# grero/HMMSpikeSorter.jl

Hardware: AMD Instinct MI355X
Metric: Msamples/sec (Viterbi + forward-backward), K=4 L=60 HMM (higher is better)
Workload: dtype f64; 1 GPU; K=4 L=60 HMM (reference N=4, K=60: 237 states), 10000000-sample single channel per GPU: one Viterbi decode + one Baum-Welch E-step (forward-backward + sufficient statistics + M-step finish); channels=1, samples_per_channel=10000000, states=237, engine=wave, block=4928, halo=295, chains=2030, seed=1234, pooled_allreduce=False

## Files before the change

### hmmspikesorter.jl_amd/csrc/wave_common.h

```cpp
#pragma once
#include <hip/hip_runtime.h>
#include <stdint.h>
#include <cmath>
#include <cstdlib>
#include <cstring>
#include <string>
#include <vector>

#include "hmmsort_internal.h"
#include "ring_common.h"

namespace hmmsort {

constexpr double kScFloor = -700.0;

struct WaveGeom {
    int64_t T;
    int C;
    int N, L;
    int W;
    int RB;
    int B;
    int Hw;
    int He;
// ... 132 lines not shown
    bool uc = true;
    int pre_rows = 0;
    bool sweeps = false;
    bool logdl = false;
    int ft = 0;
    bool gs = false;
    int gsum = kGsumNone;
    int nt = 0, ngrp = 0;
    bool decode = false;
    bool redo = false;
    bool tight = false;
    bool light = false;
    int spw = 0;
};

inline WavePick wave_pick(const WaveDev *r, int call)
{
    const WaveGeom &g = r->g;
    const int N = g.N, L = g.L;
    WavePick p;
    p.N = N; p.call = call;
    p.uc = r->uniform_cx || N > kWaveMaxPerSource;
    p.pre_rows = wave_pre_rows(N);
    p.sweeps = call != kWaveCallDecode;
    p.decode = call == kWaveCallDecode || call == kWaveCallDecodeEstep;
    if (p.sweeps) {
        p.logdl = N > 8;
        p.gs = call == kWaveCallPosteriors;
        const bool generic = getenv("HMMSORT_GSUM_GENERIC") != nullptr;
        const bool fuse4 = N == 3 || N == 4, fuse8 = N >= 5 && N <= 8;
        const bool sep = generic || p.gs || getenv("HMMSORT_GSUM_SEPARATE") != nullptr;
        p.ft = sep ? 0 : (fuse4 && L <= 64) ? 1 : (fuse8 && r->uniform_cx && L <= 64) ? 2
               : (fuse8 && r->uniform_cx && L <= 128) ? 4 : 0;
        if (p.gs) p.gsum = kGsumNone;
        else if (p.ft > 0) p.gsum = kGsumFused;
        else if (generic) p.gsum = kGsumGeneric;
        else {
            static const int nt_big = getenv("HMMSORT_GSUM_TILES") ? atoi(getenv("HMMSORT_GSUM_TILES")) : 16;
            const int want = nt_big >= 16 ? 16 : (nt_big >= 8 ? 8 : 4);
            const int np = N <= 1 ? 1 : (N <= 2 ? 2 : (N <= 4 ? 4 : (N <= 8 ? 8 : 16)));
            const int lpt = 16 * (16 / np);
            const int ntx = (L + lpt - 1) / lpt;
            p.gsum = kGsumMx;
            p.nt = N > 8 ? (ntx <= 4 ? 4 : (ntx <= 8 ? (want < 8 ? want : 8) : want)) : (ntx < 4 ? ntx : 4);
            p.ngrp = (ntx + p.nt - 1) / p.nt;
        }
    }
    if (p.decode) {
        const bool beside = call == kWaveCallDecodeEstep;
        p.redo = g.nch > 1;
        p.tight = N <= 4 && beside;
        p.light = g.backtrace == 2 || (g.backtrace == 0 && beside);
        p.spw = wave_bt_spw(N);
    }
    return p;
}

__device__ __forceinline__ double wave_bcast(double v, int lane)
{
    const int lo = __builtin_amdgcn_readlane(__double2loint(v), lane);
    const int hi = __builtin_amdgcn_readlane(__double2hiint(v), lane);
    return __hiloint2double(hi, lo);
}

template <int CTRL, int ROWMASK>
__device__ __forceinline__ double dpp_mov(double old, double v)
{
    const int lo = __builtin_amdgcn_update_dpp(__double2loint(old), __double2loint(v), CTRL, ROWMASK, 0xF, false);
    const int hi = __builtin_amdgcn_update_dpp(__double2hiint(old), __double2hiint(v), CTRL, ROWMASK, 0xF, false);
    return __hiloint2double(hi, lo);
}

__device__ __forceinline__ double lane_prev(double v, double carry)
{
    return dpp_mov<0x138, 0xF>(carry, v);
}

__device__ __forceinline__ void scan_maxplus(double &a, double &b)
{
#define HS_MP_STEP(CTRL, RM)                                                      \
    {                                                                             \
        const double al = dpp_mov<CTRL, RM>(0.0, a), bl = dpp_mov<CTRL, RM>(-INFINITY, b); \
        b = fmax(bl + a, b);                                                      \
        a = al + a;                                                               \
    }
    HS_MP_STEP(0x111, 0xF) HS_MP_STEP(0x112, 0xF) HS_MP_STEP(0x114, 0xF) HS_MP_STEP(0x118, 0xF)
    HS_MP_STEP(0x142, 0xA) HS_MP_STEP(0x143, 0xC)
#undef HS_MP_STEP
}

template <int CTRL, int ROWMASK>
__device__ __forceinline__ float dpp_movf(float old, float v)
{
    return __int_as_float(__builtin_amdgcn_update_dpp(__float_as_int(old), __float_as_int(v), CTRL, ROWMASK, 0xF, false));
}
__device__ __forceinline__ void scan_maxplus_f32(float &a, float &b)
{
#define HS_MPF_STEP(CTRL, RM)                                                     \
    {                                                                             \
        const float al = dpp_movf<CTRL, RM>(0.0f, a), bl = dpp_movf<CTRL, RM>(-INFINITY, b); \
        b = fmaxf(bl + a, b);                                                     \
        a = al + a;                                                               \
    }
    HS_MPF_STEP(0x111, 0xF) HS_MPF_STEP(0x112, 0xF) HS_MPF_STEP(0x114, 0xF) HS_MPF_STEP(0x118, 0xF)
    HS_MPF_STEP(0x142, 0xA) HS_MPF_STEP(0x143, 0xC)
#undef HS_MPF_STEP
}
__device__ __forceinline__ float lane_prevf(float v, float carry)
{
    return dpp_movf<0x138, 0xF>(carry, v);
}

__device__ __forceinline__ void scan_linear(double &a, double &b)
{
#define HS_LN_STEP(CTRL, RM)                                                      \
    {                                                                             \
        const double al = dpp_mov<CTRL, RM>(1.0, a), bl = dpp_mov<CTRL, RM>(0.0, b); \
        b = __builtin_fma(a, bl, b);                                              \
        a = al * a;                                                               \
    }
    HS_LN_STEP(0x111, 0xF) HS_LN_STEP(0x112, 0xF) HS_LN_STEP(0x114, 0xF) HS_LN_STEP(0x118, 0xF)
    HS_LN_STEP(0x142, 0xA) HS_LN_STEP(0x143, 0xC)
#undef HS_LN_STEP
}

__device__ __forceinline__ double lane_prev_ref(double v, double carry, int lane)
{
    const double s = __shfl_up(v, 1);
    return lane == 0 ? carry : s;
}
__device__ __forceinline__ void scan_maxplus_ref(double &a, double &b, int lane)
{
#pragma unroll
    for (int d = 1; d < 64; d <<= 1) {
        const double al = __shfl_up(a, d), bl = __shfl_up(b, d);
        if (lane >= d) { b = fmax(bl + a, b); a = al + a; }
    }
}
__device__ __forceinline__ void scan_linear_ref(double &a, double &b, int lane)
{
#pragma unroll
    for (int d = 1; d < 64; d <<= 1) {
        const double al = __shfl_up(a, d), bl = __shfl_up(b, d);
        if (lane >= d) { b = __builtin_fma(a, bl, b); a = al * a; }
    }
}

__device__ __forceinline__ const WaveConst *reload_consts(const WaveConst *p)
{
    asm volatile("" : "+s"(p));
    return p;
}

template <int N> constexpr int wave_depth() { return N <= 4 ? 4 : (N <= 8 ? 3 : 2); }
template <int N> constexpr int wave_occ() { return N <= 4 ? 4 : (N <= 8 ? 2 : 1); }

__device__ __forceinline__ double wave_max(double v)
{
#pragma unroll
    for (int o = 32; o > 0; o >>= 1) v = fmax(v, __shfl_xor(v, o));
    return v;
}
__device__ __forceinline__ double wave_sum(double v)
{
#pragma unroll
    for (int o = 32; o > 0; o >>= 1) v += __shfl_xor(v, o);
    return v;
}

__device__ __forceinline__ void wave_lds_order()
{
    __builtin_amdgcn_fence(__ATOMIC_RELEASE, "wavefront");
    __builtin_amdgcn_wave_barrier();
    __builtin_amdgcn_fence(__ATOMIC_ACQUIRE, "wavefront");
}

constexpr int kTieBlk = 512;
constexpr int kTieCap = 65536;
constexpr int kTieWalk = 8192;
constexpr int kTieLanes = 64;
constexpr int kTieTrig = 0;
constexpr int kTieListed = 1;
constexpr int kTieDone = 2;
constexpr int kTieFlips = 3;
constexpr int kTieOpen = 4;
constexpr int kTieTail = 5;
constexpr int kTieLongest = 6;
constexpr int kTieSerial = 7;

__device__ __forceinline__ double wpath_lp(int N, int L, const double *__restrict__ ctab, int xp, int xc)
{
    if (xp == 1) return xc == 1 ? ctab[0] : ctab[1 + (xc - 2) / L];
    const int a = (xp - 2) / L, k = (xp - 2) % L + 1;
    if (k < L) return ctab[1 + 2 * N + N * N + a * L + k];
    if (xc == 1) return ctab[1 + N + a];
    return ctab[1 + 2 * N + a * N + (xc - 2) / L];
}

__device__ __forceinline__ double wave_thr(const WaveGeom &g, const WaveConst &K, const double *__restrict__ ysum, int ch)
{
    const double T = (double)g.T;
    const double s1 = ysum[2 * ch], s2 = ysum[2 * ch + 1];
    const double sq = fmax((s2 - 2.0 * K.mean0 * s1) + T * K.mean0 * K.mean0, 0.0);
    const double mmax = fabs(K.A) * T + sq / K.den + fabs(K.c00) * T + 1.0;
    return (ldexp(16.0 * (double)(g.L + 2), ilogb(mmax) - 52) + 4.0e-9) * g.thr_scale;
}

template <typename F>
int wave_graphed(WaveDev *r, int kind, const void *p0, const void *p1, const void *p2, const void *p3,
                 hipStream_t st, F enqueue)
{
    if (!r->graphs_on || r->prof_on || st == nullptr) return enqueue(st);
    uint64_t key[12] = {(uint64_t)kind, (uint64_t)(uintptr_t)p0, (uint64_t)(uintptr_t)p1, (uint64_t)(uintptr_t)p2,
                        (uint64_t)(uintptr_t)p3, (uint64_t)(uintptr_t)st, (uint64_t)(r->bound_y == p0),
                        (uint64_t)r->uniform_cx, (uint64_t)r->g.own_lo, (uint64_t)r->g.own_hi,
                        (uint64_t)(r->g.first * 2 + r->g.last), (uint64_t)(uint32_t)r->g.tie_debug};
    {
        uint64_t tb;
        static_assert(sizeof(tb) == sizeof(r->g.thr_scale), "");
        memcpy(&tb, &r->g.thr_scale, sizeof(tb));
        key[11] ^= tb << 8;
    }
    for (auto &e : r->graphs)
        if (!memcmp(e.key, key, sizeof(key))) {
            HS_HIP(hipGraphLaunch(e.exec, st));
            return HMMSORT_OK;
        }
    if (hipStreamBeginCapture(st, hipStreamCaptureModeRelaxed) != hipSuccess) {
        (void)hipGetLastError();
        r->graphs_on = false;
        return enqueue(st);
    }
    const int rc = enqueue(st);
    hipGraph_t graph = nullptr;
    const hipError_t e1 = hipStreamEndCapture(st, &graph);
    hipGraphExec_t exec = nullptr;
    if (rc || e1 != hipSuccess || !graph || hipGraphInstantiate(&exec, graph, nullptr, nullptr, 0) != hipSuccess) {
        (void)hipGetLastError();
        if (graph) (void)hipGraphDestroy(graph);
        r->graphs_on = false;
        return rc ? rc : enqueue(st);
    }
    (void)hipGraphDestroy(graph);
    if (r->graphs.size() >= 16) {
        (void)hipGraphExecDestroy(r->graphs.front().exec);
        r->graphs.erase(r->graphs.begin());
    }
    WaveDev::GraphEntry ge;
    memcpy(ge.key, key, sizeof(key));
    ge.exec = exec;
    r->graphs.push_back(ge);
    HS_HIP(hipGraphLaunch(exec, st));
    return HMMSORT_OK;
}

inline size_t wave_zero_bytes(const WaveDev *r, bool decode)
{
    return (size_t)(decode ? 8 + 8 * (int64_t)r->g.C + 2 : 8) * sizeof(int64_t);
}

int wave_create(WaveDev **out, const std::vector<HostModel> &models, int64_t T, int64_t block_req,
                int64_t halo_req);
int wave_set_model(WaveDev *r, int ch, const HostModel &m);
void wave_destroy(WaveDev *r);
int wave_prepare(WaveDev *r, const double *d_y, hipStream_t st);
int wave_bind(WaveDev *r, const double *d_y, hipStream_t st);
int64_t wave_stats_len(const WaveDev *r);
int wave_diagnostics(WaveDev *r, hipStream_t st, int64_t diag[8]);
int wave_profile_read(WaveDev *r, hipStream_t st, std::vector<std::string> &names,
                      std::vector<double> &ms, std::vector<int64_t> &calls);
int wave_viterbi_sweep(WaveDev *r, const double *d_y, hipStream_t st);
int wave_viterbi_post(WaveDev *r, const double *d_y, int16_t *d_x, double *d_ll, hipStream_t st, bool beside);
int wave_viterbi(WaveDev *r, const double *d_y, int16_t *d_x, double *d_ll, hipStream_t st);
int wave_tie_resolve(WaveDev *r, const double *d_y, int16_t *d_x, hipStream_t st);
int wave_tie_stats(WaveDev *r, hipStream_t st, int64_t out[8]);
int wave_estep(WaveDev *r, const double *d_y, double *d_stats, hipStream_t st);
int wave_mstep(WaveDev *r, const double *d_stats, double *d_out, hipStream_t st);
int wave_decode_estep(WaveDev *r, const double *d_y, int16_t *d_x, double *d_ll, double *d_stats,
                      hipStream_t st);
int wave_post_sweeps(WaveDev *r, const double *d_y, hipStream_t st);
int wave_posteriors(WaveDev *r, const double *d_y, double *d_onset, double *d_occ, double *d_silent, double *d_logz,
                    hipStream_t st);
int wave_post_decode(WaveDev *r, int16_t *d_xm, hipStream_t st);
int wave_spike_conf(WaveDev *r, int ch, int a, int qv, int64_t jitter, const int64_t *d_times, int64_t n,
                    double *d_conf, hipStream_t st);
int wave_expected_counts(WaveDev *r, double *counts_out, hipStream_t st);

}
```

### hmmspikesorter.jl_amd/csrc/wave_estep.hip

```cpp
#include <cmath>
#include <type_traits>

#include "fastmath.h"
#include "wave_common.h"

namespace hmmsort {

constexpr double kLn2 = 6.93147180559945286227e-01;
typedef double wg_d4 __attribute__((ext_vector_type(4)));

__device__ __forceinline__ double scale_of(double v, double s)
{
    return v > 0.0 ? s + (double)ilogb(v) * kLn2 : -INFINITY;
}

template <int N>
struct FIn {
    double y;
    double R[N];
};

template <int N>
__device__ __forceinline__ void excl_sums(const double (&t)[N], double (&out)[N])
{
    double pre = 0.0;
#pragma unroll
    for (int a = 0; a < N; a++) { out[a] = pre; pre += t[a]; }
    double suf = 0.0;
#pragma unroll
    for (int a = N - 1; a >= 0; a--) { out[a] += suf; suf += t[a]; }
}

template <int N, bool UC>
__global__ __launch_bounds__(64, N <= 4 ? 3 : (N <= 8 ? 2 : 1)) void kw_fwd(WaveGeom g, const WaveConst *__restrict__ cst,
                                                            const double *__restrict__ y,
                                                            const double *__restrict__ Rf,
                                                            const double *__restrict__ virt,
                                                            double *__restrict__ FA0, double *__restrict__ FV,
                                                            double *__restrict__ FREF, double *__restrict__ fpre,
                                                            double *__restrict__ trash)
{
    constexpr int D = wave_depth<N>();
    constexpr int KSC = 5, KCP0 = 5 + N, KPEND = 5 + 2 * N, KCPX = 5 + 3 * N, KSIZE = 5 + 3 * N + N * N;
    extern __shared__ double lds[];
    const int L = g.L, W = g.W, RB = g.RB, B = g.B;
    constexpr bool LOGDL = N > 8;
    double *KC = lds, *DLv = lds + KSIZE, *DLs = LOGDL ? DLv : lds + KSIZE + N * (RB + 1);
    const int lane = threadIdx.x;
    const int cg = blockIdx.x, ch = cg / g.nch, c = cg % g.nch;
    const int64_t T = g.T;
    const int64_t tc = (int64_t)c * B;
    const int nc = (int)((T - tc) < B ? (T - tc) : B);
    const int64_t tend = tc + nc;
    const double *yc = y + (int64_t)ch * T;
    const double *Rc = Rf + (int64_t)ch * N * T;
    double *FAc = FA0 + (int64_t)ch * T, *FRc = FREF + (int64_t)ch * T, *FVc = FV + (int64_t)ch * N * T;
    const int64_t FR = 1 + (int64_t)L * (N + 1);
    double *rec = fpre + cg * FR;

    if (LOGDL) for (int i = lane; i < N * (RB + 1); i += 64) DLv[i] = -INFINITY;
    else for (int i = lane; i < 2 * N * (RB + 1); i += 64) DLv[i] = 0.0;
    {
        const WaveConst &Kg = cst[ch];
        if (lane == 0) { KC[0] = Kg.sc0; KC[1] = Kg.mean0; KC[2] = 1.0 / Kg.den; KC[3] = Kg.P00; KC[4] = fexp(-Kg.sc0); }
        if (lane < N) { KC[KSC + lane] = Kg.sc[lane]; KC[KCP0 + lane] = Kg.CP0[lane]; KC[KPEND + lane] = Kg.PEND[lane]; }
        if (UC) { if (lane < N) KC[KCPX + lane] = Kg.CPXin[lane]; }
        else for (int i = lane; i < N * N; i += 64) KC[KCPX + i] = Kg.CPXT[i];
    }
    __syncthreads();
    int64_t tinit;
    double M, x = 1.0;
    if (c == 0) {
        tinit = 0;
        for (int i = lane; i < N * L; i += 64) {
            const int a = i / L, j = i % L + 1;
            if (j < L) {
                if (!LOGDL) DLv[a * (RB + 1) + (L - j)] = 1.0;
                DLs[a * (RB + 1) + (L - j)] = virt[((int64_t)ch * N + a) * (L + 1) + j];
            }
        }
        const double d0 = yc[0] - KC[1];
        const double q00 = -((d0 * d0) * KC[2]);
        M = (double)(float)q00;
        x = fexp(q00 - M);
        if (lane < N) {
            const double f0 = fexp(-KC[KSC + lane]);
            if (LOGDL) DLs[lane * (RB + 1) + L] = Rc[(int64_t)lane * T];
            else {
                DLv[lane * (RB + 1) + L] = f0;
                DLs[lane * (RB + 1) + L] = KC[KSC + lane] + Rc[(int64_t)lane * T];
            }
            FVc[(int64_t)lane * T] = f0;
        }
        if (lane == 0) { FAc[0] = q00; FRc[0] = 0.0; }
    } else {
        tinit = tc - g.Hw;
        M = 0.0;
    }
    __syncthreads();

    const int n_total = (int)(tend - 1 - tinit);
    auto load = [&](FIn<N> &d, int off) {
        const int nact = n_total - off < W ? n_total - off : W;
        const int li = lane < nact ? lane : 0;
        int64_t tb = tinit + 1 + off;
        tb = tb < T ? tb : T - 1;
        d.y = (yc + tb)[li];
#pragma unroll
        for (int a = 0; a < N; a++) d.R[a] = (Rc + (int64_t)a * T + tb)[li];
    };
    int rs = (1 + lane) % RB, ws = (L + 1 + lane) % RB;
    auto run = [&](const FIn<N> &d, int off, auto mode_tag) {
        constexpr int MODE = decltype(mode_tag)::value;
        const int nact = n_total - off < W ? n_total - off : W;
        const bool live = lane < nact;
        const int64_t tb = tinit + 1 + off;
        const int64_t t = tb + lane;
        const double sc0 = KC[0];
        double v[N], E[N + 1];
        double e = -INFINITY;
#pragma unroll
        for (int a = 0; a < N; a++) {
            if (LOGDL) {
                v[a] = 1.0;
                E[a] = live ? DLs[a * (RB + 1) + rs] + sc0 : -INFINITY;
                e = fmax(e, E[a]);
            } else {
                v[a] = live ? DLv[a * (RB + 1) + rs] : 0.0;
                E[a] = DLs[a * (RB + 1) + rs] + sc0;
                e = fmax(e, scale_of(v[a], E[a]));
            }
        }
        const double dd = d.y - KC[1];
        const double q0 = -((dd * dd) * KC[2]);
        float fa = live ? (float)(sc0 + q0) : 0.0f;
        float fb = live ? (float)(e + q0) : -INFINITY;
        scan_maxplus_f32(fa, fb);
        const float Mf = (float)M;
        const float Mtf = fmaxf(Mf + fa, fb);
        const double Mt = (double)Mtf;
        const double Mprev = (double)lane_prevf(Mtf, Mf);
        const double ref = Mt - q0;
        E[N] = (Mprev + sc0) - ref;
#pragma unroll
        for (int a = 0; a < N; a++) E[a] = v[a] > 0.0 ? fmin(E[a] - ref, 700.0) : -INFINITY;
        fexp_n<N + 1>(E);
        const double E0 = E[N];
        double Ea[N];
        double al = E0 * KC[3], be = 0.0;
#pragma unroll
        for (int a = 0; a < N; a++) {
            Ea[a] = LOGDL ? E[a] : v[a] * E[a];
            be = __builtin_fma(Ea[a], KC[KPEND + a], be);
        }
        al = live ? al : 1.0;
        be = live ? be : 0.0;
        scan_linear(al, be);
        const double xt = __builtin_fma(al, x, be);
        const double xprev = lane_prev(xt, x);
        const double einv = KC[4];
        const double base = (xprev * E0) * einv;
        double u[N];
        if (UC) {
            double tb_[N], ex[N];
#pragma unroll
            for (int a = 0; a < N; a++) tb_[a] = Ea[a] * einv;
            excl_sums<N>(tb_, ex);
#pragma unroll
            for (int a = 0; a < N; a++) u[a] = __builtin_fma(ex[a], KC[KCPX + a], base * KC[KCP0 + a]);
        } else {
#pragma unroll
            for (int a = 0; a < N; a++) {
                double su = base * KC[KCP0 + a];
#pragma unroll
                for (int b = 0; b < N; b++)
                    if (b != a) su = __builtin_fma(Ea[b] * einv, KC[KCPX + a * N + b], su);
                u[a] = su;
                __builtin_amdgcn_sched_barrier(0);
            }
        }
        const int wsl = live ? ws : RB;
        if (LOGDL) {
            double lu[N];
#pragma unroll
            for (int a = 0; a < N; a++) lu[a] = u[a];
            flog_n<N>(lu);
#pragma unroll
            for (int a = 0; a < N; a++) DLs[a * (RB + 1) + wsl] = ((ref + KC[KSC + a]) + d.R[a]) + (u[a] > 0.0 ? lu[a] : -INFINITY);
        } else {
#pragma unroll
            for (int a = 0; a < N; a++) {
                DLv[a * (RB + 1) + wsl] = u[a];
                DLs[a * (RB + 1) + wsl] = (ref + KC[KSC + a]) + d.R[a];
            }
        }
        if (MODE == 1) {
            const double la0 = Mt + flog(xt);
            *(live ? FAc + tb + lane : trash + lane) = la0;
            *(live ? FRc + tb + lane : trash + 64 + lane) = ref;
#pragma unroll
            for (int a = 0; a < N; a++) *(live ? FVc + (int64_t)a * T + tb + lane : trash + 64 * (2 + a) + lane) = u[a];
        }
        if (MODE == 2) {
            if (live && t >= tc - L && t < tc) {
                const int64_t jj = t - (tc - L);
#pragma unroll
                for (int a = 0; a < N; a++) rec[1 + jj * (N + 1) + a] = u[a];
                rec[1 + jj * (N + 1) + N] = ref;
                if (t == tc - 1) rec[0] = Mt + flog(xt);
            }
        }
        x = wave_bcast(xt, nact - 1);
        M = wave_bcast(Mt, nact - 1);
        const int ee = x > 0.0 ? ilogb(x) : 0;
        if (ee >= 32 || ee <= -32) {
            const double Mx = M + (double)ee * kLn2, Mn = (double)(float)Mx;
            x = ldexp(x, -ee) * fexp(Mx - Mn);
            M = Mn;
        }
        rs += W; rs = rs >= RB ? rs - RB : rs;
        ws += W; ws = ws >= RB ? ws - RB : ws;
    };
    auto sweep = [&](int from, int to, auto mode_tag) {
        FIn<N> buf[D];
#pragma unroll
        for (int i = 0; i < D; i++) load(buf[i], from + i * W);
        int off = from;
        for (; off + D * W <= to; off += D * W) {
#pragma unroll
            for (int i = 0; i < D; i++) {
                run(buf[i], off + i * W, mode_tag);
                load(buf[i], off + (i + D) * W);
            }
        }
#pragma unroll
        for (int i = 0; i < D; i++)
            if (off + i * W < to) run(buf[i], off + i * W, mode_tag);
    };
    const int n_warm = c == 0 ? 0 : g.Hw - 1;
    const int n_rec = ((L + W - 1) / W) * W < n_warm ? ((L + W - 1) / W) * W : n_warm;
    if (n_warm - n_rec > 0) sweep(0, n_warm - n_rec, std::integral_constant<int, 0>());
    if (n_rec > 0) sweep(n_warm - n_rec, n_warm, std::integral_constant<int, 2>());
    sweep(n_warm, n_total, std::integral_constant<int, 1>());
}

template <int N>
struct BIn {
    double y1, y0;
    double w2;
    double R[N];
    double fv[N];
    double fref, la0;
};

constexpr int bwd_yring(int ft) { return ft <= 2 ? 256 : 512; }

#ifndef HS_BWD_W4
#define HS_BWD_W4 2
#endif
#ifndef HS_BWD_FEED
#define HS_BWD_FEED 1
#endif
#ifndef HS_BWD_ILOAD
#define HS_BWD_ILOAD 1
#endif
#ifndef HS_BWD_IPRED
#define HS_BWD_IPRED 1
#endif
constexpr int bwd_np(int n) { return n <= 4 ? 4 : 8; }
constexpr int bwd_d0(int n) { return 16 * (16 / bwd_np(n) - 1); }
constexpr int bwd_ymir(int n) { return bwd_d0(n) + 20; }
constexpr int bwd_rmir(int n) { return bwd_d0(n); }
constexpr bool bwd_feed(int ft) { return HS_BWD_FEED && ft == 1; }
constexpr int bwd_stat_doubles(int n, int ft)
{
    const int np = bwd_np(n), rpad = n <= 4 ? 1 : 2, ym = bwd_yring(ft);
    if (ft <= 0) return 0;
    if (!bwd_feed(ft)) return ym + (128 + 8 * rpad) * np;
    const int re = 128 + bwd_rmir(n);
    return (ym + bwd_ymir(n) + 2) + (re + rpad * (re >> 4) + 1) * np;
}
template <int N, bool UC, int FT = 0, bool GS = false>
__global__ __launch_bounds__(64, N <= 4 ? HS_BWD_W4 : 1) void kw_bwd(WaveGeom g, const WaveConst *__restrict__ cst,
                                                            const double *__restrict__ y,
                                                            const double *__restrict__ Rf,
                                                            const double *__restrict__ FA0,
                                                            const double *__restrict__ FV,
                                                            const double *__restrict__ FREF,
                                                            const double *__restrict__ fpre,
                                                            const double *__restrict__ W2,
                                                            double *__restrict__ rho, double *__restrict__ partS,
                                                            double *__restrict__ Zc, double *__restrict__ bpre,
                                                            double *__restrict__ bown, double *__restrict__ yhead,
                                                            double *__restrict__ trash, double *__restrict__ partG,
                                                            double *__restrict__ gsil)
{
    constexpr bool FUSE = FT > 0;
    static_assert(!GS || !FUSE, "the silent posterior is stored by the unfused sweep");
    static_assert(!FUSE || (N >= 3 && N <= 8), "the fused statistics are written for delayed copies of 3-8 rings");
    static_assert(!FUSE || N > 4 || FT == 1, "3-4 rings: one tile of 64 lags");
    constexpr int NPc = bwd_np(N), NSc = 16 / NPc, LPT = 16 * NSc;
    constexpr int RPAD = NPc == 4 ? 1 : 2;
    constexpr int RGROWS = 128 + 8 * RPAD;
    constexpr int YM = bwd_yring(FT);
    constexpr int NACC = FT <= 1 ? 2 : FT;
#ifndef HS_BWD_D4
#define HS_BWD_D4 2
#endif
    constexpr int D = N <= 4 ? HS_BWD_D4 : (N <= 8 ? 2 : 1);
    constexpr int KSC = 4, KCP0 = 4 + N, KPEND = 4 + 2 * N, KCPX = 4 + 3 * N, KSIZE = 4 + 3 * N + N * N;
    extern __shared__ double lds[];
    const int L = g.L, W = g.W, RB = g.RB, B = g.B;
    double *KC = lds, *DLv = lds + KSIZE, *DLs = lds + KSIZE + N * (RB + 1);
    const int lane = threadIdx.x;
    const int cg = blockIdx.x, ch = cg / g.nch, c = cg % g.nch;
    const int64_t T = g.T;
    const int64_t tc = (int64_t)c * B;
    const int nc = (int)((T - tc) < B ? (T - tc) : B);
    const int64_t tend = tc + nc, tstar = tend - 1;
    const int64_t te = (tend + g.He) < T ? (tend + g.He) : T;
    const double *yc = y + (int64_t)ch * T;
    const double *Rc = Rf + (int64_t)ch * N * T;
    const double *FAc = FA0 + (int64_t)ch * T, *FRc = FREF + (int64_t)ch * T, *FVc = FV + (int64_t)ch * N * T;
    double *rhoc = rho + (int64_t)ch * N * T;
    const double *W2c = W2 + (int64_t)ch * T;
    const int64_t FR = 1 + (int64_t)L * (N + 1);
    const double la0pre = c > 0 ? fpre[cg * FR] : 0.0;
    double *recp = bpre + cg * FR, *reco = bown + cg * FR;
    double *yh = yhead + (int64_t)ch * (N * L + 2);

    for (int i = lane; i < N * (RB + 1); i += 64) DLv[i] = 1.0;
    for (int i = lane; i < RB + 1; i += 64) DLs[i] = 0.0;
    double *YY = DLs + (RB + 1), *RG = YY + (bwd_feed(FT) ? YM + bwd_ymir(N) + 2 : YM);
    const int lk = lane >> 4, lj = lane & 15, gla = lj % NPc, glsft = lj / NPc;
    wg_d4 cacc[NACC > 0 ? NACC : 1];
#pragma unroll
    for (int q = 0; q < NACC; q++) cacc[q] = wg_d4{0.0, 0.0, 0.0, 0.0};
    int gtau = -1;
    auto rgrow = [&](int r) { return (r + RPAD * (r >> 4)) * NPc; };
    constexpr bool FEED = bwd_feed(FT);
    constexpr int YMIR = bwd_ymir(N), RMIR = bwd_rmir(N), RE = 128 + RMIR;
    const double *RGl = RG + (rgrow(lk - 16 * glsft + RMIR) + gla);
    const double *YYl = YY + (lk - lj + (YMIR - 16 * (NSc - 1) - 4));
    auto ystore = [&](int sigma, double v) {
        const int i = sigma & (YM - 1);
        if constexpr (FEED) {
            YY[YMIR + i] = v;
            YY[i >= YM - YMIR ? i - (YM - YMIR) : YM + YMIR] = v;
        } else YY[i] = v;
    };
    auto rstore = [&](int sigma, const double (&v)[NPc]) {
        const int r = sigma & 127;
        if constexpr (FEED) {
            double *p0 = RG + rgrow(RMIR + r), *p1 = RG + rgrow(r >= 128 - RMIR ? r - (128 - RMIR) : RE);
#pragma unroll
            for (int a = 0; a < NPc; a++) p0[a] = v[a];
#pragma unroll
            for (int a = 0; a < NPc; a++) p1[a] = v[a];
        } else {
            double *p0 = RG + rgrow(r);
#pragma unroll
            for (int a = 0; a < NPc; a++) p0[a] = v[a];
        }
    };
    auto gmfma = [&](int upto) {
        if constexpr (FEED) {
            for (; gtau + 8 <= upto; gtau += 8) {
                const int s0 = rgrow(gtau & 127), s1 = rgrow((gtau + 4) & 127), sy = (gtau + 4) & (YM - 1);
                const double b0 = RGl[s0], b1 = RGl[s1];
                const double a0 = YYl[sy], a1 = YYl[sy + 4];
                cacc[0] = __builtin_amdgcn_mfma_f64_16x16x4f64(a0, b0, cacc[0], 0, 0, 0);
                cacc[1] = __builtin_amdgcn_mfma_f64_16x16x4f64(a1, b1, cacc[1], 0, 0, 0);
            }
            if (gtau + 4 <= upto) {
                const int s0 = rgrow(gtau & 127), sy = (gtau + 4) & (YM - 1);
                const double b0 = RGl[s0];
                const double a0 = YYl[sy];
                cacc[0] = __builtin_amdgcn_mfma_f64_16x16x4f64(a0, b0, cacc[0], 0, 0, 0);
                gtau += 4;
            }
        } else if constexpr (FT <= 1) {
            constexpr int D0 = 16 * (NSc - 1);
            for (; gtau + 8 <= upto; gtau += 8) {
                const int r0 = (gtau + lk - 16 * glsft) & 127, r1 = (gtau + 4 + lk - 16 * glsft) & 127;
                const double b0 = RG[rgrow(r0) + gla], b1 = RG[rgrow(r1) + gla];
                const double a0 = YY[(gtau + lk - D0 - lj) & (YM - 1)], a1 = YY[(gtau + 4 + lk - D0 - lj) & (YM - 1)];
                cacc[0] = __builtin_amdgcn_mfma_f64_16x16x4f64(a0, b0, cacc[0], 0, 0, 0);
                cacc[1] = __builtin_amdgcn_mfma_f64_16x16x4f64(a1, b1, cacc[1], 0, 0, 0);
            }
            if (gtau + 4 <= upto) {
                const int r0 = (gtau + lk - 16 * glsft) & 127;
                const double b0 = RG[rgrow(r0) + gla];
                const double a0 = YY[(gtau + lk - D0 - lj) & (YM - 1)];
                cacc[0] = __builtin_amdgcn_mfma_f64_16x16x4f64(a0, b0, cacc[0], 0, 0, 0);
                gtau += 4;
            }
// ... 835 lines not shown
```

### hmmspikesorter.jl_amd/csrc/wave_viterbi.hip

```cpp
#include <algorithm>
#include <cmath>
#include <type_traits>

#include "wave_common.h"

namespace hmmsort {

constexpr double kVitTol = 1e-9;

template <int N>
struct WIn {
    double y;
    double R[N];
};

template <int N, bool UC, bool redo>
__device__ __forceinline__ void vit_chain(const WaveGeom &g, const WaveConst *__restrict__ cst,
                                          const double *__restrict__ y, const double *__restrict__ Rf,
                                          const double *__restrict__ virt, const double *__restrict__ ysum,
                                          uint32_t *__restrict__ psi, double *__restrict__ vpre,
                                          double *__restrict__ vend, uint32_t *__restrict__ trash, const int cg)
{
    constexpr int EB = wpsi_bits_c(N), EPW = wpsi_epw_c(N), PW = wpsi_words_c(N), D = wave_depth<N>();
    constexpr int KC0 = 3, KCEND = 3 + N, KCXT = 3 + 2 * N, KSIZE = 3 + 2 * N + N * N;
    extern __shared__ double lds_vit[];
    double *KC = lds_vit;
    double *DL = lds_vit + KSIZE;
    const int lane = threadIdx.x;
    const int ch = cg / g.nch, c = cg % g.nch;
    const int L = g.L, W = g.W, RB = g.RB, B = g.B;
    const int64_t T = g.T;
    const int64_t tc = (int64_t)c * B;
    const int nc = (int)((T - tc) < B ? (T - tc) : B);
    const int64_t tend = tc + nc;
    const double *yc = y + (int64_t)ch * T;
    const double *Rc = Rf + (int64_t)ch * N * T;
    uint32_t *psic = psi + (int64_t)ch * T;
    const int64_t SR = 1 + N * L;
    const int64_t planePsi = (int64_t)g.C * T;
    const double thr = wave_thr(g, cst[ch], ysum, ch);

    for (int i = lane; i < N * (RB + 1); i += 64) DL[i] = -INFINITY;
    {
        const WaveConst &Kg = cst[ch];
        if (lane == 0) { KC[0] = Kg.c00; KC[1] = Kg.mean0; KC[2] = Kg.den; }
        if (lane < N) { KC[KC0 + lane] = Kg.c0[lane]; KC[KCEND + lane] = Kg.cend[lane]; }
        if (UC) { if (lane < N) KC[KCXT + lane] = Kg.cxin[lane]; }
        else for (int i = lane; i < N * N; i += 64) KC[KCXT + i] = Kg.cxT[i];
    }
    __syncthreads();
    int64_t tinit;
    double D0;
    if (redo) {
        tinit = tc - 1;
        D0 = vend[(cg - 1) * SR];
        for (int i = lane; i < N * L; i += 64) {
            const int a = i / L, j = i % L + 1;
            DL[a * (RB + 1) + (L + 1 - j)] = vend[(cg - 1) * SR + 1 + i];
        }
    } else if (c == 0) {
        tinit = 0;
        D0 = -cst[ch].A;
        for (int i = lane; i < N * L; i += 64) {
            const int a = i / L, j = i % L + 1;
            DL[a * (RB + 1) + (L - j)] = virt[((int64_t)ch * N + a) * (L + 1) + j];
        }
        if (lane < N) DL[lane * (RB + 1) + L] = Rc[(int64_t)lane * T];
    } else {
        tinit = tc - g.Hw;
        D0 = 0.0;
    }
    __syncthreads();

    const int n_total = (int)(tend - 1 - tinit);
    auto load = [&](WIn<N> &d, int off) {
        const int nact = n_total - off < W ? n_total - off : W;
        const int li = lane < nact ? lane : 0;
        int64_t tb = tinit + 1 + off;
        tb = tb < T ? tb : T - 1;
        d.y = (yc + tb)[li];
#pragma unroll
        for (int a = 0; a < N; a++) d.R[a] = (Rc + (int64_t)a * T + tb)[li];
    };
    int rs = (1 + lane) % RB, ws = (L + 1 + lane) % RB;
    auto run = [&](const WIn<N> &d, int off, auto store_tag) {
        constexpr int STORE = decltype(store_tag)::value;
        const int nact = n_total - off < W ? n_total - off : W;
        const bool live = lane < nact;
        const int64_t tb = tinit + 1 + off;
        double X[N];
#pragma unroll
        for (int a = 0; a < N; a++) {
            const double v = DL[a * (RB + 1) + rs];
            X[a] = live ? v : -INFINITY;
        }
        double e1 = -INFINITY, e2 = -INFINITY;
        int earg = 0;
#pragma unroll
        for (int a = 0; a < N; a++) {
            const double v = X[a] + KC[KCEND + a];
            earg = v > e1 ? a + 1 : earg;
            e2 = fmax(e2, fmin(e1, v));
            e1 = fmax(e1, v);
        }
        const double c00 = KC[0];
        const double dd = d.y - KC[1];
        const double q0 = -((dd * dd) / KC[2]);
        double sa = live ? c00 + q0 : 0.0;
        double sb = live ? e1 + q0 : -INFINITY;
        scan_maxplus(sa, sb);
        const double Dn = fmax(D0 + sa, sb);
        const double Dprev = lane_prev(Dn, D0);
        uint32_t pw[PW];
#pragma unroll
        for (int w = 0; w < PW; w++) pw[w] = 0u;
        {
            const double v0 = Dprev + c00;
            const bool ring = e1 > v0;
            const double gap = ring ? e1 - fmax(e2, v0) : v0 - e1;
            const uint32_t fl = gap < thr ? 1u : 0u;
            pw[0] = (ring ? (uint32_t)earg : 0u) | (fl << (EB - 1));
        }
        double m1 = -INFINITY, m2 = -INFINITY, m3 = -INFINITY;
        int i1 = 0, i2 = 0;
        if (UC) {
#pragma unroll
            for (int b = 0; b < N; b++) {
                const double v = X[b];
                const bool g1 = v > m1, g2 = v > m2;
                m3 = g2 ? m2 : fmax(m3, v);
                i2 = g1 ? i1 : (g2 ? b + 1 : i2);
                m2 = g1 ? m1 : (g2 ? v : m2);
                i1 = g1 ? b + 1 : i1;
                m1 = g1 ? v : m1;
            }
        }
        const int wsl = live ? ws : RB;
#pragma unroll
        for (int a = 0; a < N; a++) {
            double r1 = -INFINITY, r2 = -INFINITY;
            int rarg = 0;
            if (UC) {
                const double cin = KC[KCXT + a];
                const bool first = (a + 1 == i1), second = (a + 1 == i2);
                r1 = (first ? m2 : m1) + cin;
                rarg = first ? i2 : i1;
                r2 = ((first || second) ? m3 : m2) + cin;
                if (N == 1) { r1 = -INFINITY; r2 = -INFINITY; rarg = 0; }
            } else {
#pragma unroll
                for (int b = 0; b < N; b++) {
                    if (b == a) continue;
                    const double v = X[b] + KC[KCXT + a * N + b];
                    rarg = v > r1 ? b + 1 : rarg;
                    r2 = fmax(r2, fmin(r1, v));
                    r1 = fmax(r1, v);
                }
            }
            const double v0 = Dprev + KC[KC0 + a];
            const bool ring = r1 > v0;
            const double u = ring ? r1 : v0;
            const double gap = ring ? r1 - fmax(r2, v0) : v0 - r1;
            const uint32_t fl = gap < thr ? 1u : 0u;
            DL[a * (RB + 1) + wsl] = u + d.R[a];
            const uint32_t ent = (ring ? (uint32_t)rarg : 0u) | (fl << (EB - 1));
            pw[(a + 1) / EPW] |= ent << (((a + 1) % EPW) * EB);
            if (!UC) __builtin_amdgcn_sched_barrier(0);
        }
        if (STORE) {
#pragma unroll
            for (int w = 0; w < PW; w++) {
                uint32_t *dst = live ? psic + w * planePsi + tb + lane : trash + lane;
                *dst = pw[w];
            }
        }
        D0 = wave_bcast(Dn, nact - 1);
        rs += W; rs = rs >= RB ? rs - RB : rs;
        ws += W; ws = ws >= RB ? ws - RB : ws;
    };
    auto dump = [&](double *rec, int64_t tref) {
        __syncthreads();
        if (lane == 0) rec[0] = D0;
        for (int i = lane; i < N * L; i += 64) {
            const int a = i / L, j = i % L + 1;
            const int slot = (int)((tref - j - tinit + L) % RB);
            rec[1 + i] = DL[a * (RB + 1) + slot];
        }
        __syncthreads();
    };
    auto sweep = [&](int from, int to, auto store_tag) {
        WIn<N> buf[D];
#pragma unroll
        for (int i = 0; i < D; i++) load(buf[i], from + i * W);
        int off = from;
        for (; off + D * W <= to; off += D * W) {
#pragma unroll
            for (int i = 0; i < D; i++) {
                run(buf[i], off + i * W, store_tag);
                load(buf[i], off + (i + D) * W);
            }
        }
#pragma unroll
        for (int i = 0; i < D; i++)
            if (off + i * W < to) run(buf[i], off + i * W, store_tag);
    };
    const int n_warm = (redo || c == 0) ? 0 : g.Hw - 1;
    if (n_warm > 0) {
        sweep(0, n_warm, std::integral_constant<int, 0>());
        dump(vpre + cg * SR, tc);
    }
    sweep(n_warm, n_total, std::integral_constant<int, 1>());
    dump(vend + cg * SR, tend);
    if (redo) {
        for (int i = lane; i < SR; i += 64) vpre[cg * SR + i] = vend[(cg - 1) * SR + i];
    }
}

template <int N, bool UC>
__global__ __launch_bounds__(64, wave_occ<N>()) void kw_vit(WaveGeom g, const WaveConst *__restrict__ cst,
                                                            const double *__restrict__ y,
                                                            const double *__restrict__ Rf,
                                                            const double *__restrict__ virt,
                                                            const double *__restrict__ ysum,
                                                            uint32_t *__restrict__ psi, double *__restrict__ vpre,
                                                            double *__restrict__ vend, uint32_t *__restrict__ trash)
{
    vit_chain<N, UC, false>(g, cst, y, Rf, virt, ysum, psi, vpre, vend, trash, (int)blockIdx.x);
}

constexpr int kVitRedoGrid = 64;
template <int N, bool UC, bool TIGHT>
__global__ __launch_bounds__(64) __attribute__((amdgpu_waves_per_eu(TIGHT ? 6 : 1))) void kw_vit_redo(WaveGeom g, const WaveConst *__restrict__ cst,
                                                                 const double *__restrict__ y,
                                                                 const double *__restrict__ Rf,
                                                                 const double *__restrict__ virt,
                                                                 const double *__restrict__ ysum,
                                                                 uint32_t *__restrict__ psi, double *__restrict__ vpre,
                                                                 double *__restrict__ vend, uint32_t *__restrict__ trash,
                                                                 const int32_t *__restrict__ head,
                                                                 const int32_t *__restrict__ list)
{
    const int n = head[0];
    for (int q = blockIdx.x; q < n; q += gridDim.x)
        vit_chain<N, UC, true>(g, cst, y, Rf, virt, ysum, psi, vpre, vend, trash, list[q]);
}

struct VitCert {
    bool fail, anybad;
    double spread;
};

__device__ __forceinline__ VitCert vit_cert(const WaveGeom &g, const double *__restrict__ vpre,
                                            const double *__restrict__ vend, int cg, int lane, double *__restrict__ dbgrec)
{
    const int c = cg % g.nch;
    const int64_t SR = 1 + (int64_t)g.N * g.L;
    double lo = INFINITY, hi = -INFINITY;
    int64_t ilo = -1, ihi = -1, ibad = -1;
    bool bad = false;
    for (int64_t i = lane; i < SR; i += 64) {
        const double p = vpre[cg * SR + i], e = vend[(cg - 1) * SR + i];
        if (p == e) {
            if (fabs(p) < INFINITY) { lo = fmin(lo, 0.0); hi = fmax(hi, 0.0); }
            continue;
        }
        const double d = p - e;
        if (!(fabs(d) < INFINITY)) { bad = true; ibad = i; continue; }
        if (d < lo) { lo = d; ilo = i; }
        if (d > hi) { hi = d; ihi = i; }
    }
    if (dbgrec) {
        for (int o = 32; o > 0; o >>= 1) {
            const double l2 = __shfl_xor(lo, o), h2 = __shfl_xor(hi, o);
            const long long il2 = __shfl_xor((long long)ilo, o), ih2 = __shfl_xor((long long)ihi, o), ib2 = __shfl_xor((long long)ibad, o);
            if (l2 < lo) { lo = l2; ilo = il2; }
            if (h2 > hi) { hi = h2; ihi = ih2; }
            if (ib2 > ibad) ibad = ib2;
        }
        if (lane == 0 && c <= 3) {
            double *r = dbgrec + 16 + 8 * (c - 1);
            r[0] = (double)cg; r[1] = lo; r[2] = (double)ilo; r[3] = hi; r[4] = (double)ihi; r[5] = (double)ibad;
            r[6] = ilo >= 0 ? vpre[cg * SR + ilo] : 0.0; r[7] = ilo >= 0 ? vend[(cg - 1) * SR + ilo] : 0.0;
        }
    }
    lo = -wave_max(-lo); hi = wave_max(hi);
    VitCert v;
    v.anybad = __any(bad);
    v.spread = hi - lo;
    v.fail = v.anybad || !(v.spread <= kVitTol);
    return v;
}

constexpr unsigned long long kVitNoSpread = ~0ull;

__device__ __forceinline__ void vit_spread_max(int64_t *__restrict__ diag, unsigned long long sb)
{
    if (sb > *reinterpret_cast<volatile unsigned long long *>(&diag[2]))
        atomicMax((unsigned long long *)&diag[2], sb);
}

__global__ __launch_bounds__(64) void kw_vit_check(WaveGeom g, const double *__restrict__ vpre,
                                                   const double *__restrict__ vend,
                                                   int32_t *__restrict__ vfail, int64_t *__restrict__ diag,
                                                   int final_round, double *__restrict__ dbg,
                                                   int32_t *__restrict__ head, int32_t *__restrict__ list,
                                                   const int32_t *__restrict__ prev_head,
                                                   unsigned long long *__restrict__ vcert)
{
    const int lane = threadIdx.x;
    const int cg = blockIdx.x, c = cg % g.nch;
    const bool same = prev_head && prev_head[0] == 0;
    if (same && !final_round) return;
    if (c == 0 && !same) { if (lane == 0) vfail[cg] = 0; return; }
    if (same) {
        if (cg % 64 == 0) {
// ... 877 lines not shown
```

Measured before the change: 11210 Msamples/s.

## Add unmasked interior sweep to forward pass and branchless top-k in Viterbi

The forward E-step kernel gains a separate interior sweep mode for chunks that are fully in bounds. That mode drops the per-lane liveness masking and index clamping, uses scalar-uniform base addresses for loads and stores, and writes FA/FR/FV outputs directly. The Viterbi kernel replaces the select-based top-3 tracking and gap computation with branchless fmax/fmin forms for N=4/7/8. The aim is fewer VALU selects and less address arithmetic in the hot loops, at the cost of more code variants and a more complex boundary calculation for the interior range.

```diff
diff --git a/hmmspikesorter.jl_amd/csrc/wave_common.h b/hmmspikesorter.jl_amd/csrc/wave_common.h
--- a/hmmspikesorter.jl_amd/csrc/wave_common.h
+++ b/hmmspikesorter.jl_amd/csrc/wave_common.h
@@ -308,6 +308,12 @@
     return p;
 }
 
+__device__ __forceinline__ int64_t uniform_base(int64_t t)
+{
+    asm volatile("" : "+s"(t));
+    return t;
+}
+
 template <int N> constexpr int wave_depth() { return N <= 4 ? 4 : (N <= 8 ? 3 : 2); }
 template <int N> constexpr int wave_occ() { return N <= 4 ? 4 : (N <= 8 ? 2 : 1); }
 
diff --git a/hmmspikesorter.jl_amd/csrc/wave_estep.hip b/hmmspikesorter.jl_amd/csrc/wave_estep.hip
--- a/hmmspikesorter.jl_amd/csrc/wave_estep.hip
+++ b/hmmspikesorter.jl_amd/csrc/wave_estep.hip
@@ -7,6 +7,10 @@
 namespace hmmsort {
 
 constexpr double kLn2 = 6.93147180559945286227e-01;
+
+#ifndef HS_FWD_INTERIOR
+#define HS_FWD_INTERIOR 1
+#endif
 typedef double wg_d4 __attribute__((ext_vector_type(4)));
 
 __device__ __forceinline__ double scale_of(double v, double s)
@@ -100,7 +104,15 @@
     __syncthreads();
 
     const int n_total = (int)(tend - 1 - tinit);
-    auto load = [&](FIn<N> &d, int off) {
+    const unsigned lin = lane < W ? (unsigned)lane : 0u;
+    auto load = [&](FIn<N> &d, int off, auto mode_tag) {
+        if constexpr (decltype(mode_tag)::value == 3) {
+            const int64_t tb = uniform_base(tinit + 1 + off);
+            d.y = (yc + tb)[lin];
+#pragma unroll
+            for (int a = 0; a < N; a++) d.R[a] = (Rc + (int64_t)a * T + tb)[lin];
+            return;
+        }
         const int nact = n_total - off < W ? n_total - off : W;
         const int li = lane < nact ? lane : 0;
         int64_t tb = tinit + 1 + off;
@@ -112,10 +124,11 @@
     int rs = (1 + lane) % RB, ws = (L + 1 + lane) % RB;
     auto run = [&](const FIn<N> &d, int off, auto mode_tag) {
         constexpr int MODE = decltype(mode_tag)::value;
-        const int nact = n_total - off < W ? n_total - off : W;
+        constexpr bool INT = MODE == 3;
+        const int nact = INT ? W : (n_total - off < W ? n_total - off : W);
         const bool live = lane < nact;
         const int64_t tb = tinit + 1 + off;
-        const int64_t t = tb + lane;
+        [[maybe_unused]] const int64_t t = tb + lane;
         const double sc0 = KC[0];
         double v[N], E[N + 1];
         double e = -INFINITY;
@@ -123,18 +136,18 @@
         for (int a = 0; a < N; a++) {
             if (LOGDL) {
                 v[a] = 1.0;
-                E[a] = live ? DLs[a * (RB + 1) + rs] + sc0 : -INFINITY;
+                E[a] = (INT || live) ? DLs[a * (RB + 1) + rs] + sc0 : -INFINITY;
                 e = fmax(e, E[a]);
             } else {
-                v[a] = live ? DLv[a * (RB + 1) + rs] : 0.0;
+                v[a] = (INT || live) ? DLv[a * (RB + 1) + rs] : 0.0;
                 E[a] = DLs[a * (RB + 1) + rs] + sc0;
                 e = fmax(e, scale_of(v[a], E[a]));
             }
         }
         const double dd = d.y - KC[1];
         const double q0 = -((dd * dd) * KC[2]);
-        float fa = live ? (float)(sc0 + q0) : 0.0f;
-        float fb = live ? (float)(e + q0) : -INFINITY;
+        float fa = (INT || live) ? (float)(sc0 + q0) : 0.0f;
+        float fb = (INT || live) ? (float)(e + q0) : -INFINITY;
         scan_maxplus_f32(fa, fb);
         const float Mf = (float)M;
         const float Mtf = fmaxf(Mf + fa, fb);
@@ -153,8 +166,10 @@
             Ea[a] = LOGDL ? E[a] : v[a] * E[a];
             be = __builtin_fma(Ea[a], KC[KPEND + a], be);
         }
-        al = live ? al : 1.0;
-        be = live ? be : 0.0;
+        if (!INT) {
+            al = live ? al : 1.0;
+            be = live ? be : 0.0;
+        }
         scan_linear(al, be);
         const double xt = __builtin_fma(al, x, be);
         const double xprev = lane_prev(xt, x);
@@ -179,7 +194,7 @@
                 __builtin_amdgcn_sched_barrier(0);
             }
         }
-        const int wsl = live ? ws : RB;
+        const int wsl = (W == 64 && INT) ? ws : (live ? ws : RB);
         if (LOGDL) {
             double lu[N];
 #pragma unroll
@@ -200,6 +215,16 @@
             *(live ? FRc + tb + lane : trash + 64 + lane) = ref;
 #pragma unroll
             for (int a = 0; a < N; a++) *(live ? FVc + (int64_t)a * T + tb + lane : trash + 64 * (2 + a) + lane) = u[a];
+        }
+        if (INT) {
+            const double la0 = Mt + flog(xt);
+            const int64_t tbu = uniform_base(tb);
+            if (live) {
+                (FAc + tbu)[(unsigned)lane] = la0;
+                (FRc + tbu)[(unsigned)lane] = ref;
+#pragma unroll
+                for (int a = 0; a < N; a++) (FVc + (int64_t)a * T + tbu)[(unsigned)lane] = u[a];
+            }
         }
         if (MODE == 2) {
             if (live && t >= tc - L && t < tc) {
@@ -224,13 +249,13 @@
     auto sweep = [&](int from, int to, auto mode_tag) {
         FIn<N> buf[D];
 #pragma unroll
-        for (int i = 0; i < D; i++) load(buf[i], from + i * W);
+        for (int i = 0; i < D; i++) load(buf[i], from + i * W, mode_tag);
         int off = from;
         for (; off + D * W <= to; off += D * W) {
 #pragma unroll
             for (int i = 0; i < D; i++) {
                 run(buf[i], off + i * W, mode_tag);
-                load(buf[i], off + (i + D) * W);
+                load(buf[i], off + (i + D) * W, mode_tag);
             }
         }
 #pragma unroll
@@ -241,7 +266,16 @@
     const int n_rec = ((L + W - 1) / W) * W < n_warm ? ((L + W - 1) / W) * W : n_warm;
     if (n_warm - n_rec > 0) sweep(0, n_warm - n_rec, std::integral_constant<int, 0>());
     if (n_rec > 0) sweep(n_warm - n_rec, n_warm, std::integral_constant<int, 2>());
-    sweep(n_warm, n_total, std::integral_constant<int, 1>());
+    int n_int = n_warm;
+    if constexpr (HS_FWD_INTERIOR) {
+        const int64_t room = T - 64 - tinit - (int64_t)n_warm - (int64_t)D * W;
+        const int64_t full = (n_total - n_warm) / W;
+        int64_t k = room / W < full ? room / W : full;
+        k = k < 0 ? 0 : k - k % D;
+        n_int = n_warm + (int)k * W;
+    }
+    if (n_int > n_warm) sweep(n_warm, n_int, std::integral_constant<int, 3>());
+    sweep(n_int, n_total, std::integral_constant<int, 1>());
 }
 
 template <int N>
diff --git a/hmmspikesorter.jl_amd/csrc/wave_viterbi.hip b/hmmspikesorter.jl_amd/csrc/wave_viterbi.hip
--- a/hmmspikesorter.jl_amd/csrc/wave_viterbi.hip
+++ b/hmmspikesorter.jl_amd/csrc/wave_viterbi.hip
@@ -7,6 +7,10 @@
 namespace hmmsort {
 
 constexpr double kVitTol = 1e-9;
+
+#ifndef HS_VIT_JUNC
+#define HS_VIT_JUNC 1
+#endif
 
 template <int N>
 struct WIn {
@@ -22,6 +26,7 @@
                                           double *__restrict__ vend, uint32_t *__restrict__ trash, const int cg)
 {
     constexpr int EB = wpsi_bits_c(N), EPW = wpsi_epw_c(N), PW = wpsi_words_c(N), D = wave_depth<N>();
+    constexpr bool JUNC = HS_VIT_JUNC && UC && (N == 4 || N == 7 || N == 8) && !redo;
     constexpr int KC0 = 3, KCEND = 3 + N, KCXT = 3 + 2 * N, KSIZE = 3 + 2 * N + N * N;
     extern __shared__ double lds_vit[];
     double *KC = lds_vit;
@@ -117,7 +122,7 @@
         {
             const double v0 = Dprev + c00;
             const bool ring = e1 > v0;
-            const double gap = ring ? e1 - fmax(e2, v0) : v0 - e1;
+            const double gap = JUNC ? fmax(e1, v0) - fmax(fmin(e1, v0), e2) : (ring ? e1 - fmax(e2, v0) : v0 - e1);
             const uint32_t fl = gap < thr ? 1u : 0u;
             pw[0] = (ring ? (uint32_t)earg : 0u) | (fl << (EB - 1));
         }
@@ -128,11 +133,19 @@
             for (int b = 0; b < N; b++) {
                 const double v = X[b];
                 const bool g1 = v > m1, g2 = v > m2;
-                m3 = g2 ? m2 : fmax(m3, v);
-                i2 = g1 ? i1 : (g2 ? b + 1 : i2);
-                m2 = g1 ? m1 : (g2 ? v : m2);
-                i1 = g1 ? b + 1 : i1;
-                m1 = g1 ? v : m1;
+                if constexpr (JUNC) {
+                    m3 = fmax(m3, fmin(m2, v));
+                    m2 = fmax(m2, fmin(m1, v));
+                    m1 = fmax(m1, v);
+                    i2 = g1 ? i1 : (g2 ? b + 1 : i2);
+                    i1 = g1 ? b + 1 : i1;
+                } else {
+                    m3 = g2 ? m2 : fmax(m3, v);
+                    i2 = g1 ? i1 : (g2 ? b + 1 : i2);
+                    m2 = g1 ? m1 : (g2 ? v : m2);
+                    i1 = g1 ? b + 1 : i1;
+                    m1 = g1 ? v : m1;
+                }
             }
         }
         const int wsl = live ? ws : RB;
@@ -159,8 +172,8 @@
             }
             const double v0 = Dprev + KC[KC0 + a];
             const bool ring = r1 > v0;
-            const double u = ring ? r1 : v0;
-            const double gap = ring ? r1 - fmax(r2, v0) : v0 - r1;
+            const double u = JUNC ? fmax(r1, v0) : (ring ? r1 : v0);
+            const double gap = JUNC ? u - fmax(fmin(r1, v0), r2) : (ring ? r1 - fmax(r2, v0) : v0 - r1);
             const uint32_t fl = gap < thr ? 1u : 0u;
             DL[a * (RB + 1) + wsl] = u + d.R[a];
             const uint32_t ent = (ring ? (uint32_t)rarg : 0u) | (fl << (EB - 1));
```

Measured after the change: 11310 Msamples/s (median of 6 runs). About the same (+0.8%).
